# LanaSina/evolutionary_illusion_generator

Measured on AMD Instinct MI355X. Metric: genome fitness evals/sec at 256x256, pop=256, higher is better.
Workload: dtype f32; 1 GPU; neat_configs/circles.txt colour pop=256, 256x256, PredNet 3,48,96,192, 21 steps, LK + rotation-symmetry score; global_pop=256, genomes_per_gpu=256, device_batch=256, structure=Circles

## Files before the change

### evolutionary_illusion_generator_amd/csrc/conv_wino4.h

```cpp
#pragma once
#include "wino_launch.h"

namespace eig {

constexpr int W4_UPOS = 256;
constexpr int W4_U_FLOATS = W4_NPOS * W4_UPOS;
constexpr int W4_NUS = 3, W4_NPS = 3;
constexpr int w4_row(bool tall) { return tall ? 28 : 40; }
constexpr int w4_ps(bool tall) { return tall ? 1024 : 768; }
constexpr int w4_pslot(bool tall) { return W4_KC * w4_ps(tall); }
constexpr int w4_p(bool tall, int k) { return tall ? k * w4_pslot(true) : (k < 2 ? k * w4_pslot(false) : 2 * w4_pslot(false) + 3 * W4_U_FLOATS); }
constexpr int w4_u(bool tall, int k) { return tall ? 3 * w4_pslot(true) + k * W4_U_FLOATS : 2 * w4_pslot(false) + k * W4_U_FLOATS; }
constexpr int w4_x(bool tall) { return tall ? w4_u(true, 0) : w4_u(false, 1); }
constexpr int W4_X_FLOATS = W4_WAVES * 2 * 4 * 64 * 4;
constexpr int wino4_lds_bytes() { return (w4_x(false) + W4_X_FLOATS) * 4; }
static_assert((w4_u(true, 2) + W4_U_FLOATS) * 4 == wino4_lds_bytes() && (w4_p(false, 2) + w4_pslot(false)) * 4 <= wino4_lds_bytes(), "LDS maps");
#ifndef EIG_W4_DEEPU
#define EIG_W4_DEEPU 1
#endif
#ifndef EIG_W4_DIAG
#define EIG_W4_DIAG 0
#endif

__device__ __forceinline__ void w4_in1d(float d0, float d1, float d2, float d3, float d4, float d5, float* T)
{
    T[0] = fmaf(4.0f, d0, fmaf(-5.0f, d2, d4));
    const float p = fmaf(-4.0f, d2, d4), q = fmaf(-4.0f, d1, d3);
    T[1] = p + q; T[2] = p - q;
    const float r = d4 - d2, s = d3 - d1;
    T[3] = fmaf(2.0f, s, r); T[4] = fmaf(-2.0f, s, r);
    T[5] = fmaf(4.0f, d1, fmaf(-5.0f, d3, d5));
}
template <int XI> __device__ __forceinline__ float w4_row(const float* d)
{
    if constexpr (XI == 0) return fmaf(4.0f, d[0], fmaf(-5.0f, d[1], d[2]));
    else if constexpr (XI == 5) return fmaf(4.0f, d[0], fmaf(-5.0f, d[1], d[2]));
    else {
        if constexpr (XI == 1) return fmaf(-4.0f, d[1], d[3]) + fmaf(-4.0f, d[0], d[2]);
        else if constexpr (XI == 2) return fmaf(-4.0f, d[1], d[3]) - fmaf(-4.0f, d[0], d[2]);
        else if constexpr (XI == 3) return fmaf(2.0f, d[2] - d[0], d[3] - d[1]);
        else return fmaf(-2.0f, d[2] - d[0], d[3] - d[1]);
    }
}
constexpr int w4_nrows(int xi) { return (xi == 0 || xi == 5) ? 3 : 4; }
constexpr int w4_rowidx(int xi, int k) { return xi == 0 ? 2 * k : xi == 5 ? 2 * k + 1 : k + 1; }
constexpr int w4_uprow(int i) { return (i + 1) >> 1; }

template <typename V4> __device__ __forceinline__ void w4_out1d(const V4& m0, const V4& m1, const V4& m2, const V4& m3, const V4& m4, const V4& m5, V4* Y)
{
    const V4 s = m1 + m2, d = m1 - m2, u = m3 + m4, w = m3 - m4;
    Y[0] = (m0 + s) + u;
    for (int e = 0; e < 4; ++e) { Y[1][e] = fmaf(2.0f, w[e], d[e]); Y[2][e] = fmaf(4.0f, u[e], s[e]); Y[3][e] = fmaf(8.0f, w[e], d[e]) + m5[e]; }
}

template <int NI, int EPI, bool TALL = false, bool HALF = false, bool PACK = false, bool NSPLIT = false>
__global__ void __launch_bounds__((HALF && !NSPLIT) ? W4_THREADS / 2 : W4_THREADS, 3) wino4_kernel(const ConvArgs a)
{
    static_assert(!NSPLIT || (HALF && NI == 4 && EPI != EPI_CONVA), "N-split: a half block, 64-column N-blocks, ConvLSTM / ConvP");
    constexpr int NIW = NSPLIT ? 2 : NI;
    constexpr bool DEEPU = HALF && EIG_W4_DEEPU;
    static_assert(!(TALL && HALF), "half blocks exist in the wide shape only");
    static_assert(!PACK || (HALF && EPI != EPI_CONVA), "packed tiles: a half block, ConvLSTM / ConvP");
    constexpr bool TGEO = TALL || PACK;
    static_assert(EPI == EPI_LSTM || EPI == EPI_CONVA || EPI == EPI_CONVP, "conv_wino4.h: ConvLSTM, ConvA, ConvP");
    static_assert(EPI != EPI_LSTM || NI == 4, "ConvLSTM: the four N-tiles are the four gates");
    static_assert(NI == 3 || NI == 4, "N-blocks of 48 or 64 columns");
    constexpr int U4 = wino4_u_floats(NI);
    constexpr int KC = W4_KC, PS = w4_ps(TGEO), W4_ROW = w4_row(TGEO);
    constexpr int W4_P0 = w4_p(TGEO, 0), W4_P1 = w4_p(TGEO, 1), W4_P2 = w4_p(TGEO, 2), W4_U0 = w4_u(TGEO, 0), W4_U1 = w4_u(TGEO, 1), W4_U2 = w4_u(TGEO, 2);
    constexpr int PK_ROWS = 18, PK_CX = 7, PK_IMG = PK_ROWS * PK_CX;
    constexpr bool WALK = !TALL && !HALF;
    constexpr int RGH = TALL ? 16 : 8;
    extern __shared__ __attribute__((aligned(16))) float lds[];
    unsigned long long tq_entry = EIG_TIMING ? __builtin_readcyclecounter() : 0;
    float* const Pb = lds;
    float* const Ub = lds;
    float* const xb = lds + w4_x(TGEO);
    const int wv_o = __builtin_amdgcn_readfirstlane((int)threadIdx.x >> 6);
    const int rg_o = HALF ? 0 : wv_o & 1, xi_o = (HALF && !NSPLIT) ? wv_o : wv_o >> 1;
    const int ng_o = NSPLIT ? wv_o & 1 : 0;
    constexpr int NWAVES = (HALF && !NSPLIT) ? W4_WAVES / 2 : W4_WAVES;
    constexpr int UPW = 36 / NWAVES;
    auto lane_id = [&]() __attribute__((always_inline)) { int l = (int)__builtin_amdgcn_mbcnt_hi(~0u, __builtin_amdgcn_mbcnt_lo(~0u, 0u)); asm volatile("" : "+v"(l)); return l; };

    const int tiles = a.tilesX * a.tilesY;
    const bool pk5 = PACK && a.tilesX == 5;
    const int ntile = PACK ? a.B + (pk5 ? (a.B + 3) >> 2 : 0) : a.B * tiles;
    const int xcd = blockIdx.x & 7, xi_ = blockIdx.x >> 3;
    auto dv = [&](int x, int d, unsigned m) __attribute__((always_inline)) { return m ? (int)__umulhi((unsigned)x, m) : x / d; };
    const int q0 = dv(xi_, a.nparts, a.mg[0]);
    const int part = xi_ - q0 * a.nparts;
    const int tlin = a.tile_map ? xcd * ((ntile + 7) >> 3) + q0 : q0 * 8 + xcd;
    if (tlin >= ntile) return;
    const int nwalk = WALK ? a.nwalk : 1, nb0 = part * nwalk;
    const bool pk_edge_o = pk5 && tlin >= a.B;
    const int eb = PACK ? (pk_edge_o ? 4 * (tlin - a.B) : tlin) : dv(tlin, tiles, a.mg[1]);
    const int t_ = PACK ? 0 : tlin - eb * tiles;
    const int tyi = dv(t_, a.tilesX, a.mg[2]), txi = t_ - tyi * a.tilesX;
    const int y0 = PACK ? 0 : tyi * (TALL ? 32 : (HALF ? 8 : 16)), x0 = PACK ? 0 : txi * (TALL ? 16 : 32);
    const int HW = a.H * a.W;

    const bool up_fused = !PACK && EPI == EPI_LSTM && a.up_src != nullptr;
    const int nkb0 = a.src[0].C / KC;
    const int nkbu = up_fused ? (a.up_C / KC) : 0;
    const bool has1 = a.nsrc > 1;
    const int nkb_o = nkb0 + nkbu + (has1 ? (a.src[1].C / KC) : 0);
    const int up_lo_o = nkb0, up_hi_o = nkb0 + nkbu;
#define EIG4_WAITCNT(imm) do { __builtin_amdgcn_s_waitcnt(imm); asm volatile("" ::: "memory"); } while (0)
#define EIG4_BARRIER() do { asm volatile("" ::: "memory"); __builtin_amdgcn_s_barrier(); asm volatile("" ::: "memory"); } while (0)
#define EIG4_LDS_BARRIER() do { EIG4_WAITCNT(0xC07F); EIG4_BARRIER(); } while (0)
#define EIG4_IS_UP(kb) ((kb) >= up_lo && (kb) < up_hi)

    typedef float f32x2 __attribute__((ext_vector_type(2)));
    constexpr unsigned W4_POSB = 4 * 16 * NI * 4;
    auto walk_body = [&](const int it) __attribute__((always_inline)) {
    const int nblk = nb0 + it;
    int zs = 0;
    asm volatile("" : "+s"(zs));
    const int wv = wv_o + zs, rg = rg_o + zs, xi = xi_o + zs, ng = ng_o + zs, nkb = nkb_o + zs, up_lo = up_lo_o + zs, up_hi = up_hi_o + zs;
    const int pch = HALF ? wv >> 1 : wv / 3, ppart = HALF ? wv & 1 : wv - pch * 3;
    const bool has_plane = !(NSPLIT && !PACK) || wv_o < 8;
    const int eb_i = eb + zs, y0_i = y0 + zs, x0_i = x0 + zs;
    const bool pk_edge = (pk_edge_o ? 1 : 0) + zs != 0;
    const unsigned long long sb0 = (unsigned long long)(a.src[0].ptr + (size_t)eb_i * a.src[0].Ct * HW);
    const unsigned long long sb1 = has1 ? (unsigned long long)(a.src[1].ptr + (size_t)eb_i * a.src[1].Ct * HW) : sb0;
    const int ist0 = a.src[0].Ct * HW * 4, ist1 = has1 ? a.src[1].Ct * HW * 4 : ist0;
    const int sz0 = a.src[0].C * HW * 4 + (PACK ? 3 * ist0 : 0), sz1 = has1 ? a.src[1].C * HW * 4 + (PACK ? 3 * ist1 : 0) : sz0;
    const int Hh = a.H >> 1, Wh = a.W >> 1, HWh = Hh * Wh;
    const unsigned long long sbu = up_fused ? (unsigned long long)(a.up_src + (size_t)eb_i * a.up_C * HWh) : sb0;
    const int szu = up_fused ? a.up_C * HWh * 4 : sz0;
    const int lane = lane_id();
    const int q = lane >> 4, col = lane & 15;
    constexpr int CPR = TALL ? 7 : 10, CREAL = TALL ? 6 : 10, NCHK = TALL ? 34 * 7 : (HALF ? 100 : 180), UROWS = TALL ? 18 : (HALF ? 6 : 10), UCHK = TALL ? 4 : 6;
    auto plane_offsets = [&](int part, int& ro, int& uo) __attribute__((always_inline)) {
        const int c = lane + 64 * part;
        const int row = c / CPR, cx = c - row * CPR;
        const int gy = y0_i - 1 + row, gx = x0_i - 4 + 4 * cx;
        ro = (c < NCHK && cx < CREAL && gy >= 0 && gy < a.H && gx >= 0 && gx < a.W) ? (gy * a.W + gx) * 4 : -1;
        const int hy = (y0_i >> 1) - 1 + row, hx = (x0_i >> 1) - 4 + 4 * cx;
        uo = (row < UROWS && cx < UCHK && hy >= 0 && hy < Hh && hx >= 0 && hx < Wh) ? (hy * Wh + hx) * 4 : -1;
    };
    int pk_ro[3] = {-1, -1, -1};
    unsigned pk_mul[3] = {0u, 0u, 0u};
    const int pk_n = (wv_o < 4 ? 2 : 1) + (NSPLIT ? 0 : 1);
    if constexpr (PACK) {
#pragma unroll
        for (int k = 0; k < 3; ++k) {
            const int c = lane + 64 * ((wv_o + NWAVES * k) & 3);
            const int p = c >= PK_IMG ? 1 : 0, c1 = c - PK_IMG * p;
            const int row = c1 / PK_CX, slot = c1 - row * PK_CX;
            const int b = slot >= 3 ? (slot >= 6 ? 2 : 1) : 0;
            const int irel = pk_edge ? 2 * p + b : 0, cx = pk_edge ? 4 + slot - 3 * b : slot;
            const int gy = row - 1, gx = 4 * cx - 4;
            const bool ok = (pk_edge ? (c < 2 * PK_IMG && b < 2) : c < PK_IMG) && eb_i + irel < a.B && gy >= 0 && gy < a.H && gx >= 0 && gx < a.W;
            pk_ro[k] = ok ? (gy * a.W + gx) * 4 : -1;
            pk_mul[k] = ok ? (unsigned)irel : 0u;
        }
    }
    int roff, uoff, roff2 = -1, uoff2 = -1;
    plane_offsets(ppart, roff, uoff);
    const bool two_parts = (TALL && wv_o < 4) || (HALF && !PACK && !NSPLIT && wv_o < 2);
    if (TALL) plane_offsets(3, roff2, uoff2);
    if (HALF) { roff2 = roff; uoff2 = uoff; }
    const int ch2 = HALF ? 3 : wv, part2 = HALF ? ppart : 3;
    auto dma_plane_at = [&](int jj, int slot_off) __attribute__((always_inline)) {
        const int j = jj < nkb ? jj : nkb - 1;
        const bool up = EIG4_IS_UP(j);
        const bool s1 = j >= up_hi;
        const unsigned long long mu = 0ull - (unsigned long long)up, m1 = 0ull - (unsigned long long)s1;
        const unsigned long long u = sb0 + ((sb1 - sb0) & m1) + ((sbu - sb0) & mu);
        const unsigned lo = __builtin_amdgcn_readfirstlane((unsigned)u), hi = __builtin_amdgcn_readfirstlane((unsigned)(u >> 32));
        const int sz = sz0 + ((sz1 - sz0) & (int)m1) + ((szu - sz0) & (int)mu);
        const __amdgpu_buffer_rsrc_t rs = __builtin_amdgcn_make_buffer_rsrc((void*)(((unsigned long long)hi << 32) | lo), 0, __builtin_amdgcn_readfirstlane(sz), 0x00020000);
        const int base = (up_lo & (int)mu) + (up_hi & (int)m1), hw = HW + ((HWh - HW) & (int)mu);
        if constexpr (PACK) {
            const unsigned ist = (unsigned)(ist0 + ((ist1 - ist0) & (int)m1));
#pragma unroll
            for (int k = 0; k < 3; ++k) {
                if (k >= pk_n) break;
                const int idx = wv_o + NWAVES * k;
                const unsigned coffk = (unsigned)((j - base) * KC + (idx >> 2)) * (unsigned)(hw * 4);
                __builtin_amdgcn_raw_ptr_buffer_load_lds(rs, (__attribute__((address_space(3))) void*)(Pb + slot_off + (idx >> 2) * PS + (idx & 3) * 256), 16,
                                                         (int)__builtin_elementwise_add_sat((unsigned)pk_ro[k] + pk_mul[k] * ist, coffk), 0, 0, 0);
            }
            return;
        }
        if (!has_plane) return;
        const unsigned coff = (unsigned)((j - base) * KC + pch) * (unsigned)(hw * 4);
        __builtin_amdgcn_raw_ptr_buffer_load_lds(rs, (__attribute__((address_space(3))) void*)(Pb + slot_off + pch * PS + ppart * 256), 16,
                                                 (int)__builtin_elementwise_add_sat((unsigned)roff + (((unsigned)uoff - (unsigned)roff) & (unsigned)mu), coff), 0, 0, 0);
        if (two_parts) {
            const unsigned coff2 = (unsigned)((j - base) * KC + ch2) * (unsigned)(hw * 4);
            __builtin_amdgcn_raw_ptr_buffer_load_lds(rs, (__attribute__((address_space(3))) void*)(Pb + slot_off + ch2 * PS + part2 * 256), 16,
                                                     (int)__builtin_elementwise_add_sat((unsigned)roff2 + (((unsigned)uoff2 - (unsigned)roff2) & (unsigned)mu), coff2), 0, 0, 0);
        }
    };
    auto wait_u = [&]() __attribute__((always_inline)) {
        const int npl = PACK ? pk_n : (two_parts ? 2 : (has_plane ? 1 : 0));
        switch (npl + (DEEPU ? UPW : 0)) {
            case 0: EIG4_WAITCNT(0x0F70); break;
            case 1: EIG4_WAITCNT(0x0F71); break;
            case 2: EIG4_WAITCNT(0x0F72); break;
            case 3: EIG4_WAITCNT(0x0F73); break;
            case 4: EIG4_WAITCNT(0x0F74); break;
            case 5: EIG4_WAITCNT(0x0F75); break;
            case 6: EIG4_WAITCNT(0x0F76); break;
            case 7: EIG4_WAITCNT(0x0F77); break;
            case 8: EIG4_WAITCNT(0x0F78); break;
            default: EIG4_WAITCNT(0x0F79); break;
        }
    };
    const int uvo = (NI == 4 || lane < 48) ? lane * 16 : -1;
    auto prologue_a = [&](int nb) __attribute__((always_inline)) {
        const __amdgpu_buffer_rsrc_t rs = __builtin_amdgcn_make_buffer_rsrc((void*)(a.wpk + (size_t)nb * nkb * U4), 0, (nkb + 1) * U4 * 4, 0x00020000);
#pragma unroll
        for (int i = 0; i < UPW; ++i)
            __builtin_amdgcn_raw_ptr_buffer_load_lds(rs, (__attribute__((address_space(3))) void*)(Ub + W4_U0 + (UPW * wv + i) * W4_UPOS), 16, uvo, (int)((unsigned)(UPW * wv + i) * W4_POSB), 0, 0);
        dma_plane_at(0, W4_P0);
        dma_plane_at(1, W4_P1);
    };
    auto prologue_b = [&](int nb) __attribute__((always_inline)) {
        const __amdgpu_buffer_rsrc_t rs = __builtin_amdgcn_make_buffer_rsrc((void*)(a.wpk + (size_t)nb * nkb * U4), 0, (nkb + 1) * U4 * 4, 0x00020000);
#pragma unroll
        for (int i = 0; i < UPW; ++i)
            __builtin_amdgcn_raw_ptr_buffer_load_lds(rs, (__attribute__((address_space(3))) void*)(Ub + W4_U1 + (UPW * wv + i) * W4_UPOS), 16, uvo,
                                                     (int)((unsigned)U4 * 4 + (unsigned)(UPW * wv + i) * W4_POSB), 0, 0);
        dma_plane_at(2, W4_P2);
    };

    const int pk_ir = pk_edge ? col >> 2 : 0, pk_ty = pk_edge ? col & 3 : col >> 2;
    const int t_ty = PACK ? 0 : (TALL ? col >> 2 : col >> 3), t_tx = PACK ? (pk_edge ? 3 * (pk_ir & 1) : col & 3) : (TALL ? col & 3 : col & 7);
    const int pk_row = PACK ? PK_ROWS * (pk_ir >> 1) + 4 * pk_ty : 0;
    const float* const pbase_n = Pb + q * PS + (RGH * rg + 4 * t_ty + pk_row) * W4_ROW + 4 * t_tx;
    const float* const pbase_u = Pb + q * PS + ((RGH / 2) * rg + 2 * t_ty) * W4_ROW + 2 * t_tx + 3;
    const int b_off = xi * 6 * W4_UPOS + (q * 16 + col) * NI + 2 * ng;

    unsigned long long tq_setup = tq_entry;
    if (it == 0) {
        if (EIG_TIMING) tq_setup = __builtin_readcyclecounter();
        prologue_a(nb0);
        EIG4_WAITCNT(0x0F70);
    }
    const __amdgpu_buffer_rsrc_t rsw = __builtin_amdgcn_make_buffer_rsrc((void*)(a.wpk + (size_t)nblk * nkb * U4), 0, (nkb + 1) * U4 * 4, 0x00020000);
    unsigned u_so = (unsigned)(UPW * wv) * W4_POSB + 2u * (unsigned)U4 * 4u;
    auto dma_u = [&](int slot_off) __attribute__((always_inline)) {
#pragma unroll
        for (int i = 0; i < UPW; ++i)
            __builtin_amdgcn_raw_ptr_buffer_load_lds(rsw, (__attribute__((address_space(3))) void*)(Ub + slot_off + (UPW * wv + i) * W4_UPOS), 16, uvo,
                                                     (int)(u_so + (unsigned)i * W4_POSB), 0, 0);
        u_so += (unsigned)U4 * 4;
    };
    f32x4 acc[6][NIW];
#pragma unroll
    for (int p = 0; p < 6; ++p)
#pragma unroll
        for (int ni = 0; ni < NIW; ++ni) acc[p][ni] = (f32x4){0.f, 0.f, 0.f, 0.f};
    EIG4_BARRIER();
    prologue_b(nblk);
    const unsigned long long tq_k0 = EIG_TIMING ? __builtin_readcyclecounter() : 0;
    unsigned long long tq_k1 = 0, tq_x = 0, tq_y = 0;
    auto timeline = [&]() __attribute__((always_inline)) {
        if (EIG_TIMING && a.dbg && lane_id() == 0) {
            unsigned hwid, xcc;
            asm volatile("s_getreg_b32 %0, hwreg(HW_REG_HW_ID)" : "=s"(hwid));
            asm volatile("s_getreg_b32 %0, hwreg(HW_REG_XCC_ID)" : "=s"(xcc));
            unsigned long long* dd = a.dbg + (((size_t)blockIdx.x * nwalk + it) * NWAVES + wv) * 8;
            const unsigned long long tq_end = __builtin_readcyclecounter();
            dd[0] = tq_entry; dd[1] = tq_setup; dd[2] = tq_k0; dd[3] = tq_k1; dd[4] = tq_x; dd[5] = tq_y; dd[6] = tq_end;
            dd[7] = (unsigned long long)hwid | ((unsigned long long)xcc << 32);
            tq_entry = tq_end;
        }
    };

    auto kloops = [&](auto role_tag) __attribute__((always_inline)) {
        constexpr int XI = decltype(role_tag)::value;
        float v[6];
        float bq[NIW];
        int uo0 = W4_U0, uo1 = W4_U1, uo2 = W4_U2;
        int po0 = W4_P0, po1 = W4_P1, po2 = W4_P2;
        int pj = 0, psz = 0, pbound = 0;
        unsigned pcoff = 0, plo = 0, phi = 0, phw4 = 0, pist = 0;
        bool pup = false;
        auto plane_source = [&](int j) __attribute__((always_inline)) {
            const bool up = EIG4_IS_UP(j);
            const bool s1 = j >= up_hi;
            const unsigned long long mu = 0ull - (unsigned long long)up, m1 = 0ull - (unsigned long long)s1;
            const unsigned long long u = sb0 + ((sb1 - sb0) & m1) + ((sbu - sb0) & mu);
            plo = __builtin_amdgcn_readfirstlane((unsigned)u); phi = __builtin_amdgcn_readfirstlane((unsigned)(u >> 32));
            psz = __builtin_amdgcn_readfirstlane(sz0 + ((sz1 - sz0) & (int)m1) + ((szu - sz0) & (int)mu));
            const int base = (up_lo & (int)mu) + (up_hi & (int)m1);
            phw4 = (unsigned)((HW + ((HWh - HW) & (int)mu)) * 4);
            pcoff = (unsigned)((j - base) * KC + (PACK ? 0 : pch)) * phw4;
            if constexpr (PACK) pist = (unsigned)(ist0 + ((ist1 - ist0) & (int)m1));
            pup = up; pj = j;
            pbound = j < up_lo ? up_lo : (j < up_hi ? up_hi : nkb);
        };
        auto dma_plane = [&]() __attribute__((always_inline)) {
            const unsigned o = (unsigned)roff + (((unsigned)uoff - (unsigned)roff) & (0u - (unsigned)pup));
            const __amdgpu_buffer_rsrc_t prs = __builtin_amdgcn_make_buffer_rsrc((void*)(((unsigned long long)phi << 32) | plo), 0, psz, 0x00020000);
            if constexpr (PACK) {
#pragma unroll
                for (int k = 0; k < 3; ++k) {
                    if (k >= pk_n) break;
                    const int idx = wv + NWAVES * k;
                    __builtin_amdgcn_raw_ptr_buffer_load_lds(prs, (__attribute__((address_space(3))) void*)(Pb + po0 + (idx >> 2) * PS + (idx & 3) * 256), 16,
                                                             (int)__builtin_elementwise_add_sat((unsigned)pk_ro[k] + pk_mul[k] * pist, pcoff + (unsigned)(idx >> 2) * phw4), 0, 0, 0);
                }
            } else if (has_plane) {
            __builtin_amdgcn_raw_ptr_buffer_load_lds(prs, (__attribute__((address_space(3))) void*)(Pb + po0 + pch * PS + ppart * 256), 16,
                                                     (int)__builtin_elementwise_add_sat(o, pcoff), 0, 0, 0);
            }
            if (two_parts) {
                const unsigned o2 = (unsigned)roff2 + (((unsigned)uoff2 - (unsigned)roff2) & (0u - (unsigned)pup));
                __builtin_amdgcn_raw_ptr_buffer_load_lds(prs, (__attribute__((address_space(3))) void*)(Pb + po0 + ch2 * PS + part2 * 256), 16,
                                                         (int)__builtin_elementwise_add_sat(o2, pcoff + (unsigned)(ch2 - pch) * phw4), 0, 0, 0);
            }
            if (__builtin_expect(pj + 1 == pbound, 0)) { if (pbound < nkb) plane_source(pj + 1); }
            else { ++pj; pcoff += KC * phw4; }
        };
        plane_source(3 < nkb ? 3 : nkb - 1);
        float pr[2][6];
        float t[6];
        int rso = 0;
        bool rup = false;
        auto read_rows = [&](int ph) __attribute__((always_inline)) {
            if (EIG_W4_DIAG & 4) return;
            constexpr bool END = XI == 0 || XI == 5;
#pragma unroll
            for (int j = 0; j < 2; ++j) {
                const int k = ph == 0 ? (END ? 1 + j : 1 + 2 * j) : (END ? 0 : 2 * j);
                if (ph == 1 && END && j == 1) continue;
                if (rup) {
                    const float* const pl = pbase_u + rso + w4_uprow(w4_rowidx(XI, k)) * W4_ROW;
                    const float s0 = pl[0], s1_ = pl[1], s2 = pl[2], s3 = pl[3];
                    pr[j][0] = s0; pr[j][1] = s1_; pr[j][2] = s1_; pr[j][3] = s2; pr[j][4] = s2; pr[j][5] = s3;
                } else {
                    const float* const pl = pbase_n + rso + w4_rowidx(XI, k) * W4_ROW;
                    typedef const volatile __attribute__((address_space(3))) f32x2* lds_f32x2;
                    const f32x2 c0 = *(lds_f32x2)(pl + 2), c2 = *(lds_f32x2)(pl + 8);
                    const f32x4 c1 = *reinterpret_cast<const f32x4*>(pl + 4);
                    pr[j][0] = c0[1]; pr[j][1] = c1[0]; pr[j][2] = c1[1]; pr[j][3] = c1[2]; pr[j][4] = c1[3]; pr[j][5] = c2[0];
                }
            }
        };
        auto rows_begin = [&](int slot_off, bool up) __attribute__((always_inline)) {
            rso = slot_off; rup = up;
            read_rows(0);
        };
        auto rows_mid = [&]() __attribute__((always_inline)) {
            if (!(EIG_W4_DIAG & 4)) {
#pragma unroll
                for (int c = 0; c < 6; ++c) {
                    if constexpr (XI == 0 || XI == 5) t[c] = fmaf(-5.0f, pr[0][c], pr[1][c]);
                    else if constexpr (XI == 1 || XI == 2) t[c] = fmaf(-4.0f, pr[0][c], pr[1][c]);
                    else t[c] = pr[1][c] - pr[0][c];
                }
            }
            read_rows(1);
        };
        auto rows_end = [&]() __attribute__((always_inline)) {
            if (EIG_W4_DIAG & 4) return;
#pragma unroll
            for (int c = 0; c < 6; ++c) {
                if constexpr (XI == 0 || XI == 5) t[c] = fmaf(4.0f, pr[0][c], t[c]);
                else if constexpr (XI == 1) t[c] = t[c] + fmaf(-4.0f, pr[0][c], pr[1][c]);
                else if constexpr (XI == 2) t[c] = t[c] - fmaf(-4.0f, pr[0][c], pr[1][c]);
                else if constexpr (XI == 3) t[c] = fmaf(2.0f, pr[1][c] - pr[0][c], t[c]);
                else t[c] = fmaf(-2.0f, pr[1][c] - pr[0][c], t[c]);
            }
        };
        auto build_cols = [&]() __attribute__((always_inline)) {
            if (EIG_W4_DIAG & 4) { for (int c = 0; c < 6; ++c) v[c] = 1.0f; return; }
            w4_in1d(t[0], t[1], t[2], t[3], t[4], t[5], v);
        };
        auto read_b = [&](int slot_off, int nu, float* dst) __attribute__((always_inline)) {
            const float* const bsrc = Ub + slot_off + b_off + nu * W4_UPOS;
            if constexpr (NSPLIT) {
                const f32x2 b2 = *reinterpret_cast<const f32x2*>(bsrc);
                dst[0] = b2[0]; dst[1] = b2[1];
            } else if constexpr (NI == 4) {
                const f32x4 b4 = *reinterpret_cast<const f32x4*>(bsrc);
                dst[0] = b4[0]; dst[1] = b4[1]; dst[2] = b4[2]; dst[3] = b4[3];
            } else {
#pragma unroll
                for (int ni = 0; ni < NI; ++ni) dst[ni] = bsrc[ni];
            }
        };
        auto kiter = [&](const int kb, auto kind_tag, auto nk_tag, auto last_tag, auto first_tag) __attribute__((always_inline)) {
            constexpr int KIND = decltype(kind_tag)::value;
            constexpr int NK = decltype(nk_tag)::value;
            constexpr bool LAST = decltype(last_tag)::value;
            constexpr bool FIRST = decltype(first_tag)::value || (DEEPU && !LAST);
            constexpr bool UP = KIND == 1;
            constexpr bool IDLE = UP && XI == 2;
            constexpr int NCH = IDLE ? 0 : (UP ? 5 : 6);
            float bv[2][NIW];
            auto slice = [&](int i) __attribute__((always_inline)) {
                if constexpr (!LAST) {
                    if (i == 0) { if (!(EIG_W4_DIAG & 16)) dma_u(uo2); }
                    if (i == 1) { if (!(EIG_W4_DIAG & 8)) dma_plane(); }
                    if (i == NCH - 4) rows_begin(po1, NK == 2 ? EIG4_IS_UP(kb + 1) : NK == 1);
                    if (i == NCH - 3) rows_mid();
                    if (i == NCH - 2) rows_end();
                    if (i == NCH - 1) build_cols();
                }
            };
            if constexpr (IDLE) {
                if constexpr (!LAST) {
                    if (!(EIG_W4_DIAG & 16)) dma_u(uo2);
                    if (!(EIG_W4_DIAG & 8)) dma_plane();
                    rows_begin(po1, NK == 2 ? EIG4_IS_UP(kb + 1) : NK == 1); rows_mid(); rows_end();
                    if constexpr (!FIRST) read_b(uo1, 0, bq);
                    build_cols();
                }
            } else {
#pragma unroll
                for (int i = 0; i < NCH; ++i) {
                    const int nu = (UP && i >= 2) ? i + 1 : i;
                    if (i + 1 < NCH) {
                        const int nu1 = (UP && i + 1 >= 2) ? i + 2 : i + 1;
                        read_b(uo0, nu1, bv[(i + 1) & 1]);
                    } else if constexpr (!LAST && !FIRST) read_b(uo1, 0, bq);
                    const float* const b = i == 0 ? bq : bv[i & 1];
#pragma unroll
                    for (int ni = 0; ni < NIW; ++ni) acc[nu][ni] = __builtin_amdgcn_mfma_f32_16x16x4f32(v[nu], b[ni], acc[nu][ni], 0, 0, 0);
                    slice(i);
                    __builtin_amdgcn_sched_barrier(0);
                }
            }
            { const int t0 = uo0; uo0 = uo1; uo1 = uo2; uo2 = t0; }
            { const int t0 = po0; po0 = po1; po1 = po2; po2 = t0; }
            if (LAST || (EIG_W4_DIAG & (8 | 16))) EIG4_WAITCNT(0x0F70);
            else if (!(EIG_W4_DIAG & 2)) { if (!(EIG_W4_DIAG & 1)) wait_u(); }
            if (!(EIG_W4_DIAG & 2) || LAST) EIG4_BARRIER();
            if constexpr (FIRST) read_b(uo0, 0, bq);
        };
        const std::false_type nl{};
        const std::integral_constant<int, 2> rt{};
        int kb = 0;
        rows_begin(W4_P0, EIG4_IS_UP(0)); rows_mid(); rows_end();
        read_b(W4_U0, 0, bq);
        build_cols();
        EIG4_WAITCNT(0xC07F);
        EIG4_BARRIER();
        auto run = [&](const int end, auto kind_tag) __attribute__((always_inline)) {
            for (; kb + 1 < end; ++kb) kiter(kb, kind_tag, kind_tag, nl, nl);
            if (kb + 1 == end && end < nkb) { kiter(kb, kind_tag, rt, nl, nl); ++kb; }
        };
        kiter(0, std::integral_constant<int, 0>{}, std::integral_constant<int, 0>{}, nl, std::true_type{});
        kb = 1;
        run(up_lo, std::integral_constant<int, 0>{});
        run(up_hi, std::integral_constant<int, 1>{});
        run(nkb, std::integral_constant<int, 0>{});
        kiter(nkb - 1, rt, rt, std::true_type{}, nl);
    };
    switch (xi) {
        case 0: kloops(std::integral_constant<int, 0>{}); break;
        case 1: kloops(std::integral_constant<int, 1>{}); break;
        case 2: kloops(std::integral_constant<int, 2>{}); break;
        case 3: kloops(std::integral_constant<int, 3>{}); break;
        case 4: kloops(std::integral_constant<int, 4>{}); break;
        default: kloops(std::integral_constant<int, 5>{}); break;
    }
    if (EIG_TIMING) tq_k1 = __builtin_readcyclecounter();
    const bool more = it + 1 < nwalk;
    if (more) prologue_a(nblk + 1);

    f32x4 cc[4][NIW];
#pragma unroll
    for (int ni = 0; ni < NIW; ++ni) {
        f32x4 Y[4];
        w4_out1d(acc[0][ni], acc[1][ni], acc[2][ni], acc[3][ni], acc[4][ni], acc[5][ni], Y);
#pragma unroll
        for (int b = 0; b < 4; ++b) cc[b][ni] = Y[b];
    }
    {
    int zf = 0;
    asm volatile("" : "+s"(zf));
    const int eb = eb_i + zf, y0 = y0_i + zf, x0 = x0_i + zf, wv = wv_o + zf, rg = rg_o + zf, xi = xi_o + zf, HWf = HW + zf, Cout = a.Cout + zf, ngf = ng_o + zf;
    const bool pk_edge_f = (pk_edge_o ? 1 : 0) + zf != 0;
    const int lane = lane_id();
    const int q = lane >> 4, col = lane & 15;
    const size_t cHW = (size_t)HWf;
    const int j = TALL ? lane & 3 : lane & 7, chl = TALL ? lane >> 2 : lane >> 3, e_r = j & 3, ql = TALL ? 0 : j >> 2;
    int woff[4];
#pragma unroll
    for (int e = 0; e < 4; ++e) woff[e] = (((2 * xi + (NSPLIT ? ngf : rg)) * 2 * 4 + e) * 64 + q * 16 + ((col + 4 * e + (PACK ? q : (TALL ? 0 : 8 * (q & 1)))) & 15)) * 4;
    const int fr = lane & 15, fchl = lane >> 4;
    const int f_i = pk_edge_f ? fr >> 2 : 0, f_ty = pk_edge_f ? fr & 3 : fr >> 2, f_tx = pk_edge_f ? 4 : fr & 3;
    if constexpr (EPI == EPI_LSTM || EPI == EPI_CONVP) {
        const int nun = NSPLIT ? ((xi < 4 && ngf == 0) ? 2 : 1) : (xi < 4 ? 3 : 2);
        auto unit_cq = [&](int un) __attribute__((always_inline)) { return xi < 4 ? (NSPLIT ? (ngf ? 2 : un) : un) : 3; };
        auto unit_arow = [&](int un) __attribute__((always_inline)) { return xi < 4 ? xi : 2 * (xi - 4) + (NSPLIT ? ngf : un); };
        int xoff[3];
#pragma unroll
        for (int un = 0; un < 3; ++un) {
            const int cq = unit_cq(un);
            const int ty = TALL ? cq : cq >> 1, chh = TALL ? 0 : cq & 1;
            xoff[un] = TALL ? (e_r * 64 + ty * 16 + ((chl + 4 * e_r) & 15)) * 4 : (e_r * 64 + (2 * ty + ql) * 16 + ((8 * chh + chl + 4 * e_r + 8 * ql) & 15)) * 4;
            if constexpr (PACK) xoff[un] = ((fr & 3) * 64 + (fr >> 2) * 16 + ((4 * cq + fchl + 4 * (fr & 3) + (fr >> 2)) & 15)) * 4;
        }
        auto finish = [&](int arow, int nr, int off, int xw) __attribute__((always_inline)) -> f32x4 {
            auto C = [&](int x) __attribute__((always_inline)) { return *reinterpret_cast<const f32x4*>(xb + ((x * 2 + xw) * 2 + nr) * 1024 + off); };
            const f32x4 c1 = C(1), c2 = C(2), c3 = C(3), c4 = C(4);
            const f32x4 s_ = c1 + c2, d_ = c1 - c2, u_ = c3 + c4, w_ = c3 - c4;
            f32x4 y;
            if (arow == 0) { const f32x4 c0 = C(0); y = (c0 + s_) + u_; }
            else if (arow == 1) { for (int b = 0; b < 4; ++b) y[b] = fmaf(2.0f, w_[b], d_[b]); }
            else if (arow == 2) { for (int b = 0; b < 4; ++b) y[b] = fmaf(4.0f, u_[b], s_[b]); }
            else { const f32x4 c5 = C(5); for (int b = 0; b < 4; ++b) y[b] = fmaf(8.0f, w_[b], d_[b]) + c5[b]; }
            return y;
        };
        f32x4 ys[NI][3];
        auto finish_unit = [&](int ni, int nr, int xw, int un) __attribute__((always_inline)) {
            const int sel = NSPLIT ? ngf : un;
            switch (xi) {
                case 0: ys[ni][un] = finish(0, nr, xoff[un], xw); break;
                case 1: ys[ni][un] = finish(1, nr, xoff[un], xw); break;
                case 2: ys[ni][un] = finish(2, nr, xoff[un], xw); break;
                case 3: ys[ni][un] = finish(3, nr, xoff[un], xw); break;
                case 4: ys[ni][un] = sel ? finish(1, nr, xoff[un], xw) : finish(0, nr, xoff[un], xw); break;
                default: ys[ni][un] = sel ? finish(3, nr, xoff[un], xw) : finish(2, nr, xoff[un], xw); break;
            }
        };
        if constexpr (NSPLIT) {
#pragma unroll
            for (int nr = 0; nr < 2; ++nr)
#pragma unroll
                for (int e = 0; e < 4; ++e) {
                    f32x4 t;
                    t[0] = cc[0][nr][e]; t[1] = cc[1][nr][e]; t[2] = cc[2][nr][e]; t[3] = cc[3][nr][e];
                    *reinterpret_cast<f32x4*>(xb + woff[e] + nr * 1024) = t;
                }
            EIG4_LDS_BARRIER();
            if (EIG_TIMING) tq_x = __builtin_readcyclecounter();
#pragma unroll
            for (int ni = 0; ni < NI; ++ni)
#pragma unroll
                for (int un = 0; un < 2; ++un) {
                    if (un >= nun) break;
                    finish_unit(ni, ni & 1, ni >> 1, un);
                }
        } else {
#pragma unroll
        for (int rnd = 0; rnd < 2; ++rnd) {
            if (2 * rnd >= NI) break;
            if (rnd) EIG4_LDS_BARRIER();
#pragma unroll
            for (int nr = 0; nr < 2; ++nr) {
                const int ni = 2 * rnd + nr;
                if (ni >= NI) break;
#pragma unroll
                for (int e = 0; e < 4; ++e) {
                    f32x4 t;
                    t[0] = cc[0][ni][e]; t[1] = cc[1][ni][e]; t[2] = cc[2][ni][e]; t[3] = cc[3][ni][e];
                    *reinterpret_cast<f32x4*>(xb + woff[e] + nr * 1024) = t;
                }
            }
            EIG4_LDS_BARRIER();
            if (EIG_TIMING && rnd == 0) tq_x = __builtin_readcyclecounter();
#pragma unroll
            for (int nr = 0; nr < 2; ++nr) {
                const int ni = 2 * rnd + nr;
                if (ni >= NI) break;
#pragma unroll
                for (int un = 0; un < 3; ++un) {
                    if (un >= nun) break;
                    finish_unit(ni, nr, rg, un);
                }
            }
        }
        }
        if (more) EIG4_WAITCNT(0x0F70);
        if (EIG_TIMING) { asm volatile("s_waitcnt lgkmcnt(0)" ::: "memory"); tq_y = __builtin_readcyclecounter(); }
#pragma unroll
        for (int un = 0; un < 3; ++un) {
            if (un >= nun) break;
            const int cq = unit_cq(un);
            const int ty = TALL ? cq : cq >> 1, chh = TALL ? 0 : cq & 1;
            const int arow = unit_arow(un);
            const int gy = PACK ? 4 * f_ty + arow : y0 + RGH * rg + 4 * ty + arow, gx = PACK ? 4 * f_tx : x0 + 4 * j;
            if (gy >= a.H || gx >= a.W) continue;
            const int ebo = PACK ? eb + f_i : eb;
            if (PACK && ebo >= a.B) continue;
            const size_t pix = (size_t)gy * a.W + gx;
            const int chq = PACK ? 4 * cq + fchl : 8 * chh + chl;
            if constexpr (EPI == EPI_LSTM) {
                const int ch = nblk * 16 + chq;
                if (ch >= Cout) continue;
                const float bi = a.bias[ch], bf = a.bias[Cout + ch], bc = a.bias[2 * Cout + ch], bo = a.bias[3 * Cout + ch];
                const size_t cbase = ((size_t)ebo * Cout + ch) * cHW, ps = (size_t)Cout * cHW, pbase = (size_t)ch * cHW;
                const f32x4 cold4 = *reinterpret_cast<const f32x4*>(a.c_state + cbase + pix);
                const f32x4 pi4 = *reinterpret_cast<const f32x4*>(a.peep + pbase + pix);
                const f32x4 pf4 = *reinterpret_cast<const f32x4*>(a.peep + ps + pbase + pix);
                const f32x4 po4 = *reinterpret_cast<const f32x4*>(a.peep + 2 * ps + pbase + pix);
                f32x4 cn4, hn4;
#pragma unroll
                for (int b = 0; b < 4; ++b) {
                    float cn, hn;
                    lstm_cell(ys[0][un][b], ys[1][un][b], ys[2][un][b], ys[3][un][b], bi, bf, bc, bo, cold4[b], pi4[b], pf4[b], po4[b], cn, hn);
                    cn4[b] = cn; hn4[b] = hn;
                }
                *reinterpret_cast<f32x4*>(a.c_state + cbase + pix) = cn4;
                *reinterpret_cast<f32x4*>(a.h_out + cbase + pix) = hn4;
            } else {
#pragma unroll
                for (int ni = 0; ni < NI; ++ni) {
                    const int ch = (nblk * NI + ni) * 16 + chq;
                    if (ch >= Cout) continue;
                    const float bb_ = a.bias[ch];
                    f32x4 v4;
#pragma unroll
                    for (int b = 0; b < 4; ++b) v4[b] = relu_f(ys[ni][un][b] + bb_);
                    *reinterpret_cast<f32x4*>(a.Pout + ((size_t)ebo * Cout + ch) * cHW + pix) = v4;
                }
            }
        }
    } else {
        const int Ho = a.H >> 1, Wo = a.W >> 1;
        const size_t plane = (size_t)Ho * Wo;
        const int ox = (x0 >> 1) + 2 * j;
#pragma unroll
        for (int rnd = 0; rnd < 2; ++rnd) {
            if (2 * rnd >= NI) break;
            const int nval = NI - 2 * rnd >= 2 ? 2 : 1;
            if (rnd) EIG4_LDS_BARRIER();
#pragma unroll
            for (int nr = 0; nr < 2; ++nr) {
                if (nr >= nval) break;
                const int ni = 2 * rnd + nr;
#pragma unroll
                for (int e = 0; e < 4; ++e) {
                    f32x4 t;
                    t[0] = cc[0][ni][e]; t[1] = cc[1][ni][e]; t[2] = cc[2][ni][e]; t[3] = cc[3][ni][e];
                    *reinterpret_cast<f32x4*>(xb + woff[e] + nr * 1024) = t;
                }
            }
            EIG4_LDS_BARRIER();
            if (rnd == (NI - 1) / 2) { if (more) EIG4_WAITCNT(0x0F70); }
            if (EIG_TIMING && rnd == 0) { tq_x = __builtin_readcyclecounter(); tq_y = tq_x; }
            const int g0 = nval == 2 ? (xi < 4 ? 3 * xi : 12 + 2 * (xi - 4)) : (xi < 2 ? 2 * xi : xi + 2);
            const int cnt = nval == 2 ? (xi < 4 ? 3 : 2) : (xi < 2 ? 2 : 1);
#pragma unroll
            for (int un = 0; un < 3; ++un) {
                if (un >= cnt) break;
                const int g = g0 + un;
                const int nr = g >> 3, ty = TALL ? (g >> 1) & 3 : (g >> 2) & 1, ap = TALL ? g & 1 : (g >> 1) & 1, chh = TALL ? 0 : g & 1;
                const int off = TALL ? ((nr + 2 * rg) * 256 + e_r * 64 + ty * 16 + ((chl + 4 * e_r) & 15)) * 4
                                     : ((nr + 2 * rg) * 256 + e_r * 64 + (2 * ty + ql) * 16 + ((8 * chh + chl + 4 * e_r + 8 * ql) & 15)) * 4;
                auto C = [&](int x) __attribute__((always_inline)) { return *reinterpret_cast<const f32x4*>(xb + x * 4096 + off); };
                const f32x4 c1 = C(1), c2 = C(2), c3 = C(3), c4 = C(4);
                const f32x4 s_ = c1 + c2, d_ = c1 - c2, u_ = c3 + c4, w_ = c3 - c4;
                f32x4 ya, yb;
                if (ap == 0) {
                    const f32x4 c0 = C(0);
                    ya = (c0 + s_) + u_;
                    for (int b = 0; b < 4; ++b) yb[b] = fmaf(2.0f, w_[b], d_[b]);
                } else {
                    const f32x4 c5 = C(5);
                    for (int b = 0; b < 4; ++b) { ya[b] = fmaf(4.0f, u_[b], s_[b]); yb[b] = fmaf(8.0f, w_[b], d_[b]) + c5[b]; }
                }
                const int ch = (nblk * NI + 2 * rnd + nr) * 16 + 8 * chh + chl;
                const int oy = (y0 >> 1) + (RGH / 2) * rg + 2 * ty + ap;
                if (oy >= Ho || ox >= Wo || ch >= Cout) continue;
                const float bb_ = a.bias[ch];
                const size_t pb = ((size_t)eb * Cout + ch) * plane + (size_t)oy * Wo + ox;
                const size_t e0 = ((size_t)eb * 2 * Cout + ch) * plane + (size_t)oy * Wo + ox, e1 = e0 + (size_t)Cout * plane;
                const f32x2 p2 = *reinterpret_cast<const f32x2*>(a.P + pb);
                f32x2 ea, eb2;
#pragma unroll
                for (int bp = 0; bp < 2; ++bp) {
                    const float v00 = relu_f(ya[2 * bp] + bb_), v01 = relu_f(ya[2 * bp + 1] + bb_);
                    const float v10 = relu_f(yb[2 * bp] + bb_), v11 = relu_f(yb[2 * bp + 1] + bb_);
                    const float A = fmaxf(fmaxf(v00, v01), fmaxf(v10, v11));
                    ea[bp] = relu_f(A - p2[bp]);
                    eb2[bp] = relu_f(p2[bp] - A);
                }
                *reinterpret_cast<f32x2*>(a.E + e0) = ea;
                *reinterpret_cast<f32x2*>(a.E + e1) = eb2;
            }
        }
    }
    }
    timeline();
    };
    for (int it = 0; it < nwalk; ++it) walk_body(it);
#undef EIG4_WAITCNT
#undef EIG4_BARRIER
#undef EIG4_LDS_BARRIER
#undef EIG4_IS_UP
}

}
```

Before: 431.0 genome evals/s.

## Trim upsampled-plane DMA and defer next-block prologue into LSTM epilogue

For the walking LSTM epilogue variant of the Winograd conv kernel, the upsampled input planes now use a compact row pitch, and waves with a nonzero plane part skip their now-redundant buffer-to-LDS loads. A custom waitcnt picks the right count depending on whether a load was issued. The next block's prologue (weights plus first input planes) is also moved out of the kernel tail and issued inside the first LSTM epilogue unit, so the loads overlap the gate math. The guarded loads, inline asm branch and changed LDS indexing add complexity and a risk of subtle layout or wait-count mistakes.

Result: slower. 422.1 genome evals/s (-2.0%).

```diff
diff --git a/evolutionary_illusion_generator_amd/csrc/conv_wino4.h b/evolutionary_illusion_generator_amd/csrc/conv_wino4.h
--- a/evolutionary_illusion_generator_amd/csrc/conv_wino4.h
+++ b/evolutionary_illusion_generator_amd/csrc/conv_wino4.h
@@ -17,6 +17,12 @@
 static_assert((w4_u(true, 2) + W4_U_FLOATS) * 4 == wino4_lds_bytes() && (w4_p(false, 2) + w4_pslot(false)) * 4 <= wino4_lds_bytes(), "LDS maps");
 #ifndef EIG_W4_DEEPU
 #define EIG_W4_DEEPU 1
+#endif
+#ifndef EIG_W4_LEAN_DMA
+#define EIG_W4_LEAN_DMA 1
+#endif
+#ifndef EIG_W4_LATE_A
+#define EIG_W4_LATE_A 1
 #endif
 #ifndef EIG_W4_DIAG
 #define EIG_W4_DIAG 0
@@ -132,13 +138,16 @@
     const int lane = lane_id();
     const int q = lane >> 4, col = lane & 15;
     constexpr int CPR = TALL ? 7 : 10, CREAL = TALL ? 6 : 10, NCHK = TALL ? 34 * 7 : (HALF ? 100 : 180), UROWS = TALL ? 18 : (HALF ? 6 : 10), UCHK = TALL ? 4 : 6;
+    constexpr bool LEAN = WALK && EPI == EPI_LSTM && EIG_W4_LEAN_DMA;
+    constexpr int UCPR = LEAN ? UCHK : CPR, W4_UROW = LEAN ? 4 * UCHK : W4_ROW;
     auto plane_offsets = [&](int part, int& ro, int& uo) __attribute__((always_inline)) {
         const int c = lane + 64 * part;
         const int row = c / CPR, cx = c - row * CPR;
         const int gy = y0_i - 1 + row, gx = x0_i - 4 + 4 * cx;
         ro = (c < NCHK && cx < CREAL && gy >= 0 && gy < a.H && gx >= 0 && gx < a.W) ? (gy * a.W + gx) * 4 : -1;
-        const int hy = (y0_i >> 1) - 1 + row, hx = (x0_i >> 1) - 4 + 4 * cx;
-        uo = (row < UROWS && cx < UCHK && hy >= 0 && hy < Hh && hx >= 0 && hx < Wh) ? (hy * Wh + hx) * 4 : -1;
+        const int urow = c / UCPR, ucx = c - urow * UCPR;
+        const int hy = (y0_i >> 1) - 1 + urow, hx = (x0_i >> 1) - 4 + 4 * ucx;
+        uo = (urow < UROWS && ucx < UCHK && hy >= 0 && hy < Hh && hx >= 0 && hx < Wh) ? (hy * Wh + hx) * 4 : -1;
     };
     int pk_ro[3] = {-1, -1, -1};
     unsigned pk_mul[3] = {0u, 0u, 0u};
@@ -186,6 +195,7 @@
             return;
         }
         if (!has_plane) return;
+        if (LEAN && up && ppart != 0) return;
         const unsigned coff = (unsigned)((j - base) * KC + pch) * (unsigned)(hw * 4);
         __builtin_amdgcn_raw_ptr_buffer_load_lds(rs, (__attribute__((address_space(3))) void*)(Pb + slot_off + pch * PS + ppart * 256), 16,
                                                  (int)__builtin_elementwise_add_sat((unsigned)roff + (((unsigned)uoff - (unsigned)roff) & (unsigned)mu), coff), 0, 0, 0);
@@ -195,7 +205,11 @@
                                                      (int)__builtin_elementwise_add_sat((unsigned)roff2 + (((unsigned)uoff2 - (unsigned)roff2) & (unsigned)mu), coff2), 0, 0, 0);
         }
     };
-    auto wait_u = [&]() __attribute__((always_inline)) {
+    auto wait_u = [&](bool plane_issued) __attribute__((always_inline)) {
+        if (LEAN) {
+            asm volatile("s_cmp_lg_u32 %0, 0\n\ts_cbranch_scc1 .Lw4_wait_u_%=\n\ts_waitcnt vmcnt(0)\n.Lw4_wait_u_%=:\n\ts_waitcnt vmcnt(1)" : : "s"((int)plane_issued) : "scc", "memory");
+            return;
+        }
         const int npl = PACK ? pk_n : (two_parts ? 2 : (has_plane ? 1 : 0));
         switch (npl + (DEEPU ? UPW : 0)) {
             case 0: EIG4_WAITCNT(0x0F70); break;
@@ -232,7 +246,7 @@
     const int t_ty = PACK ? 0 : (TALL ? col >> 2 : col >> 3), t_tx = PACK ? (pk_edge ? 3 * (pk_ir & 1) : col & 3) : (TALL ? col & 3 : col & 7);
     const int pk_row = PACK ? PK_ROWS * (pk_ir >> 1) + 4 * pk_ty : 0;
     const float* const pbase_n = Pb + q * PS + (RGH * rg + 4 * t_ty + pk_row) * W4_ROW + 4 * t_tx;
-    const float* const pbase_u = Pb + q * PS + ((RGH / 2) * rg + 2 * t_ty) * W4_ROW + 2 * t_tx + 3;
+    const float* const pbase_u = Pb + q * PS + ((RGH / 2) * rg + 2 * t_ty) * W4_UROW + 2 * t_tx + 3;
     const int b_off = xi * 6 * W4_UPOS + (q * 16 + col) * NI + 2 * ng;
 
     unsigned long long tq_setup = tq_entry;
@@ -281,6 +295,7 @@
         int pj = 0, psz = 0, pbound = 0;
         unsigned pcoff = 0, plo = 0, phi = 0, phw4 = 0, pist = 0;
         bool pup = false;
+        bool pissued = true;
         auto plane_source = [&](int j) __attribute__((always_inline)) {
             const bool up = EIG4_IS_UP(j);
             const bool s1 = j >= up_hi;
@@ -307,8 +322,10 @@
                                                              (int)__builtin_elementwise_add_sat((unsigned)pk_ro[k] + pk_mul[k] * pist, pcoff + (unsigned)(idx >> 2) * phw4), 0, 0, 0);
                 }
             } else if (has_plane) {
-            __builtin_amdgcn_raw_ptr_buffer_load_lds(prs, (__attribute__((address_space(3))) void*)(Pb + po0 + pch * PS + ppart * 256), 16,
-                                                     (int)__builtin_elementwise_add_sat(o, pcoff), 0, 0, 0);
+                pissued = !(LEAN && pup && ppart != 0);
+                if (pissued)
+                    __builtin_amdgcn_raw_ptr_buffer_load_lds(prs, (__attribute__((address_space(3))) void*)(Pb + po0 + pch * PS + ppart * 256), 16,
+                                                             (int)__builtin_elementwise_add_sat(o, pcoff), 0, 0, 0);
             }
             if (two_parts) {
                 const unsigned o2 = (unsigned)roff2 + (((unsigned)uoff2 - (unsigned)roff2) & (0u - (unsigned)pup));
@@ -331,7 +348,7 @@
                 const int k = ph == 0 ? (END ? 1 + j : 1 + 2 * j) : (END ? 0 : 2 * j);
                 if (ph == 1 && END && j == 1) continue;
                 if (rup) {
-                    const float* const pl = pbase_u + rso + w4_uprow(w4_rowidx(XI, k)) * W4_ROW;
+                    const float* const pl = pbase_u + rso + w4_uprow(w4_rowidx(XI, k)) * W4_UROW;
                     const float s0 = pl[0], s1_ = pl[1], s2 = pl[2], s3 = pl[3];
                     pr[j][0] = s0; pr[j][1] = s1_; pr[j][2] = s1_; pr[j][3] = s2; pr[j][4] = s2; pr[j][5] = s3;
                 } else {
@@ -431,7 +448,7 @@
             { const int t0 = uo0; uo0 = uo1; uo1 = uo2; uo2 = t0; }
             { const int t0 = po0; po0 = po1; po1 = po2; po2 = t0; }
             if (LAST || (EIG_W4_DIAG & (8 | 16))) EIG4_WAITCNT(0x0F70);
-            else if (!(EIG_W4_DIAG & 2)) { if (!(EIG_W4_DIAG & 1)) wait_u(); }
+            else if (!(EIG_W4_DIAG & 2)) { if (!(EIG_W4_DIAG & 1)) wait_u(pissued); }
             if (!(EIG_W4_DIAG & 2) || LAST) EIG4_BARRIER();
             if constexpr (FIRST) read_b(uo0, 0, bq);
         };
@@ -463,8 +480,9 @@
         default: kloops(std::integral_constant<int, 5>{}); break;
     }
     if (EIG_TIMING) tq_k1 = __builtin_readcyclecounter();
+    constexpr bool LATE_A = WALK && EPI == EPI_LSTM && EIG_W4_LATE_A;
     const bool more = it + 1 < nwalk;
-    if (more) prologue_a(nblk + 1);
+    if (!LATE_A) { if (more) prologue_a(nblk + 1); }
 
     f32x4 cc[4][NIW];
 #pragma unroll
@@ -571,8 +589,26 @@
             }
         }
         }
-        if (more) EIG4_WAITCNT(0x0F70);
+        if (!LATE_A) { if (more) EIG4_WAITCNT(0x0F70); }
         if (EIG_TIMING) { asm volatile("s_waitcnt lgkmcnt(0)" ::: "memory"); tq_y = __builtin_readcyclecounter(); }
+        auto prologue_a_late = [&](int nb) __attribute__((always_inline)) {
+            const int ln = lane_id();
+            const int nkbf = nkb_o + zf, pchf = wv / 3, ppf = wv - 3 * pchf;
+            const __amdgpu_buffer_rsrc_t rs = __builtin_amdgcn_make_buffer_rsrc((void*)(a.wpk + (size_t)nb * nkbf * U4), 0, (nkbf + 1) * U4 * 4, 0x00020000);
+            const int uvo_l = (NI == 4 || ln < 48) ? ln * 16 : -1;
+#pragma unroll
+            for (int i = 0; i < UPW; ++i)
+                __builtin_amdgcn_raw_ptr_buffer_load_lds(rs, (__attribute__((address_space(3))) void*)(Ub + W4_U0 + (UPW * wv + i) * W4_UPOS), 16, uvo_l, (int)((unsigned)(UPW * wv + i) * W4_POSB), 0, 0);
+            const int c = ln + 64 * ppf;
+            const int row = c / 10, cx = c - row * 10;
+            const int py = y0 - 1 + row, px = x0 - 4 + 4 * cx;
+            const int ro = (c < 180 && py >= 0 && py < a.H && px >= 0 && px < a.W) ? (py * a.W + px) * 4 : -1;
+            const __amdgpu_buffer_rsrc_t ps = __builtin_amdgcn_make_buffer_rsrc((void*)(a.src[0].ptr + (size_t)eb * a.src[0].Ct * HWf), 0, a.src[0].C * HWf * 4, 0x00020000);
+#pragma unroll
+            for (int jj = 0; jj < 2; ++jj)
+                __builtin_amdgcn_raw_ptr_buffer_load_lds(ps, (__attribute__((address_space(3))) void*)(Pb + (jj ? W4_P1 : W4_P0) + pchf * PS + ppf * 256), 16,
+                                                         (int)__builtin_elementwise_add_sat((unsigned)ro, (unsigned)(jj * KC + pchf) * (unsigned)(HWf * 4)), 0, 0, 0);
+        };
 #pragma unroll
         for (int un = 0; un < 3; ++un) {
             if (un >= nun) break;
@@ -580,12 +616,47 @@
             const int ty = TALL ? cq : cq >> 1, chh = TALL ? 0 : cq & 1;
             const int arow = unit_arow(un);
             const int gy = PACK ? 4 * f_ty + arow : y0 + RGH * rg + 4 * ty + arow, gx = PACK ? 4 * f_tx : x0 + 4 * j;
-            if (gy >= a.H || gx >= a.W) continue;
+            if (!LATE_A && (gy >= a.H || gx >= a.W)) continue;
             const int ebo = PACK ? eb + f_i : eb;
             if (PACK && ebo >= a.B) continue;
             const size_t pix = (size_t)gy * a.W + gx;
             const int chq = PACK ? 4 * cq + fchl : 8 * chh + chl;
-            if constexpr (EPI == EPI_LSTM) {
+            if constexpr (EPI == EPI_LSTM && LATE_A) {
+                const int ch = nblk * 16 + chq;
+                const bool ok = gy < a.H && gx < a.W && ch < Cout;
+                const size_t cbase = ((size_t)ebo * Cout + ch) * cHW, ps = (size_t)Cout * cHW, pbase = (size_t)ch * cHW;
+                float bi = 0.f, bf = 0.f, bc = 0.f, bo = 0.f;
+                f32x4 cold4 = {0.f, 0.f, 0.f, 0.f}, pi4 = cold4, pf4 = cold4, po4 = cold4;
+                if (ok) {
+                    bi = a.bias[ch]; bf = a.bias[Cout + ch]; bc = a.bias[2 * Cout + ch]; bo = a.bias[3 * Cout + ch];
+                    cold4 = *reinterpret_cast<const f32x4*>(a.c_state + cbase + pix);
+                    pi4 = *reinterpret_cast<const f32x4*>(a.peep + pbase + pix);
+                    pf4 = *reinterpret_cast<const f32x4*>(a.peep + ps + pbase + pix);
+                    po4 = *reinterpret_cast<const f32x4*>(a.peep + 2 * ps + pbase + pix);
+                }
+                f32x4 cn4, hn4;
+                auto gates = [&]() __attribute__((always_inline)) {
+#pragma unroll
+                    for (int b = 0; b < 4; ++b) {
+                        float cn, hn;
+                        lstm_cell(ys[0][un][b], ys[1][un][b], ys[2][un][b], ys[3][un][b], bi, bf, bc, bo, cold4[b], pi4[b], pf4[b], po4[b], cn, hn);
+                        cn4[b] = cn; hn4[b] = hn;
+                    }
+                };
+                if (un == 0 && more) {
+                    __builtin_amdgcn_sched_barrier(0);
+                    prologue_a_late(nblk + 1);
+                    __builtin_amdgcn_sched_barrier(0);
+                    gates();
+                    EIG4_WAITCNT(0x0F70);
+                } else {
+                    gates();
+                }
+                if (ok) {
+                    *reinterpret_cast<f32x4*>(a.c_state + cbase + pix) = cn4;
+                    *reinterpret_cast<f32x4*>(a.h_out + cbase + pix) = hn4;
+                }
+            } else if constexpr (EPI == EPI_LSTM) {
                 const int ch = nblk * 16 + chq;
                 if (ch >= Cout) continue;
                 const float bi = a.bias[ch], bf = a.bias[Cout + ch], bc = a.bias[2 * Cout + ch], bo = a.bias[3 * Cout + ch];
```
